# bepu/bepuphysics2

Hardware: NVIDIA H100
Metric: constraint-iterations/sec (solver+integrator) (higher is better)
Workload: dtype f32

## Files before the change

bepuphysics2_b200/csrc/bepu_device_types.h:

```cpp
#pragma once
#include <cuda_runtime.h>
#include <stdint.h>

namespace bepucuda {

constexpr uint32_t kRefIndexMask = 0x0FFFFFFFu;
constexpr uint32_t kRefBundleIntegratesBit = 1u << 28;
constexpr uint32_t kRefIntegrateBit = 1u << 29;
constexpr uint32_t kRefKinematicBit = 1u << 30;
constexpr int32_t kRefEmpty = -1;

struct BodyBuffers {
    float4* pose;
    float4* velocity;
    float4* inertia_local;
    float4* inertia_world;
    const uint8_t* constrained;
    int32_t count;
};

struct DeviceTypeBatch {
    int32_t type_id;
    int32_t bundle_count;
    int32_t device_batch;
    int32_t pad;
    int32_t* refs;
    float* prestep;
    float* impulses;
};

struct FrameParams {
    float dt;
// ... 64 lines not shown
```

bepuphysics2_b200/csrc/bepu_integration.cuh:

```cuda
#pragma once
#include "bepu_device_math.cuh"

namespace BEPU_NS {

BEPU_DI Q4 integrate_orientation(Q4 start, V3 w, float halfDt) {
    float speed = length(w);
    float halfAngle = speed * halfDt;
    float s = sin_approx(halfAngle);
    float scl = s / speed;
    Q4 q{w.x * scl, w.y * scl, w.z * scl, cos_approx(halfAngle)};
    Q4 end = normalize(concatenate(start, q));
    return speed > 1e-15f ? end : start;
}
BEPU_DI Sym3 rotate_inverse_inertia(Sym3 local, Q4 q) { return rotation_sandwich(matrix_from_quaternion(q), local); }
BEPU_DI void callback_integrate_velocity(Velocity& v, float gx, float gy, float gz, float linearDampingDt, float angularDampingDt) {
    v.lin = (v.lin + V3{gx, gy, gz}) * linearDampingDt;
    v.ang = v.ang * angularDampingDt;
}
BEPU_DI void integrate_velocity_extensions(Velocity& v, bool accelerations, V3 linearAcceleration, V3 angularAcceleration, float dt, bool pointGravity, V3 position,
                                           V3 center, float attractorDt) {
    if (accelerations) {
        v.lin = v.lin + linearAcceleration * dt;
        v.ang = v.ang + angularAcceleration * dt;
    }
    if (pointGravity) {
        const V3 offset = position - center;
        const float distance = length(offset);
        const float inverse = 1.0f / fmaxf(1.0f, distance * distance * distance);
        v.lin = v.lin - (offset * attractorDt) * inverse;
// ... 39 lines not shown
```

bepuphysics2_b200/csrc/bepu_layout_kernels.h:

```cpp
#pragma once
#include "bepu_device_types.h"

namespace bepucuda {

void launch_split_bodies(const void* raw, int body_count, const BodyBuffers& B, cudaStream_t s);
void launch_merge_bodies(void* raw, int body_count, const BodyBuffers& B, cudaStream_t s);
struct TransposeDesc {
    int32_t* src_refs;
    float* src_prestep;
    float* src_impulses;
    const int32_t* map;
    int32_t src_count;
    int32_t bodies, prestep_rows, impulse_rows;
    int32_t src_bundle_base;
    int32_t flags;
    const int32_t* features_old;
    const int32_t* features_new;
};
constexpr int32_t kDescResidentImpulses = 1, kDescRedistribute = 2;
enum { kTransposeRefs = 1, kTransposePrestep = 2, kTransposeImpulses = 4 };
void launch_transpose_in_all(const DeviceTypeBatch* tbs, const TransposeDesc* descs, const WorkItem* work, int work_count, int W, int what, cudaStream_t s);
void launch_transpose_out_all(const DeviceTypeBatch* tbs, const TransposeDesc* descs, const WorkItem* work, int work_count, int W, int what, cudaStream_t s);
void launch_fill_i32(int32_t* p, size_t n, int32_t v, cudaStream_t s);
void launch_redistribute_impulses(const DeviceTypeBatch* tbs, const TransposeDesc* descs, const WorkItem* work, int work_count, cudaStream_t s);
// ... 5 lines not shown
    size_t bytes;
};
void launch_batched_copy(const CopyChunk* chunks, int chunk_count, cudaStream_t s);
void launch_ownership_pass1(const DeviceTypeBatch* tbs, const WorkItem* work, int work_count, const int32_t* bodies_per_type, int sync_batch_count, int body_count,
                            int32_t* first_batch, int32_t* sync_refcount, unsigned long long* sync_mask, int32_t* error_flag, cudaStream_t s);
void launch_ownership_rest(const DeviceTypeBatch* tbs, const WorkItem* work, int work_count, const int32_t* bodies_per_type, int body_count, const int32_t* first_batch,
                           const int32_t* sync_refcount, const unsigned long long* sync_mask, uint8_t* constrained, const int32_t* kinematics, int kinematic_count,
                           int32_t* error_flag, const TransposeDesc* descs, int W, int32_t* source_bundle_flags, cudaStream_t s);
void launch_shard_barrier(const ShardPeers& peers, const FrameParams* fp, uint32_t exchange_index, int32_t* error_flag, cudaStream_t s);

void launch_fill_peer_masks(const int32_t* refs, uint32_t* peer_masks, size_t count, const uint8_t* body_masks, int rank, cudaStream_t s);
void launch_boundary_flags(const WorkRecord* records, int count, const int32_t* bodies_per_type, long long peer_delta, uint8_t* flags, cudaStream_t s);

void launch_pack_ref_rows(const WorkRecord* records, int count, int32_t* rows, cudaStream_t s);

constexpr int kLaunchPdl = 1, kLaunchPrefetchRows = 2, kLaunchIntegratorExtensions = 4, kLaunchContactsOnly = 8, kLaunchPrefetchBodies = 16;
struct ShardLaunch {
    ShardPeers peers;
    long long peer_delta;
    ShardStage stage;
};
struct SolverLaunchers {
    void (*constraint_stage)(int stage, const WorkRecord* records, const int32_t* ref_rows, int work_count, const BodyBuffers& B, const FrameParams* fp, int launch_flags,
                             const ShardLaunch* shard, cudaStream_t s);
    void (*kinematic_stage)(int stage, const int32_t* kinematics, int count, const BodyBuffers& B, const FrameParams* fp, int launch_flags, cudaStream_t s);
    void (*final_pose)(const BodyBuffers& B, const FrameParams* fp, int launch_flags, cudaStream_t s);
};
const SolverLaunchers* get_launchers_bepu_fast();
const SolverLaunchers* get_launchers_bepu_strict();

}
// ... 1 lines not shown
```

bepuphysics2_b200/csrc/bepu_solver_kernels.cu:

```cuda
#include <atomic>
#include "bepu_solver_kernels.cuh"
#include "bepu_layout_kernels.h"

namespace BEPU_NS {

using StageLauncher = void(const WorkRecord* records, const int32_t* ref_rows, int work_count, const BodyBuffers& B, const FrameParams* fp, int launch_flags,
                           const ShardLaunch* shard, cudaStream_t s);
StageLauncher launch_stage_warm_start_first, launch_stage_warm_start, launch_stage_solve;

#ifndef BEPU_DEEP_MINB
#define BEPU_DEEP_MINB 12
#endif
constexpr int kDeepBatchBundles = 2150;
#ifndef BEPU_CONTACT_MINB
#define BEPU_CONTACT_MINB 10
#endif
#ifndef BEPU_CONTACT_SOLVE_MINB
#define BEPU_CONTACT_SOLVE_MINB 12
#endif
template <auto Kernel, class... Args>
static void launch_stage_kernel(int work_count, int launch_flags, cudaStream_t s, Args... args) {
    static std::atomic<bool> carveout_set[64] = {};
    int device = 0;
    cudaGetDevice(&device);
    if (!carveout_set[device & 63]) {
        cudaFuncSetAttribute(Kernel, cudaFuncAttributePreferredSharedMemoryCarveout, cudaSharedmemCarveoutMaxShared);
        carveout_set[device & 63] = true;
    }
    const unsigned blocks = (unsigned)(((size_t)work_count * 32 + kStageBlockThreads - 1) / kStageBlockThreads);
    cudaLaunchConfig_t cfg{};
    cfg.gridDim = dim3(blocks);
    cfg.blockDim = dim3(kStageBlockThreads);
    cfg.stream = s;
    cudaLaunchAttribute attr[1];
    attr[0].id = cudaLaunchAttributeProgrammaticStreamSerialization;
    attr[0].val.programmaticStreamSerializationAllowed = 1;
    cfg.attrs = attr;
    cfg.numAttrs = (launch_flags & bepucuda::kLaunchPdl) ? 1 : 0;
    cudaLaunchKernelEx(&cfg, Kernel, args...);
}
template <int STAGE, int MINB, bool kExt, bool kContacts>
static void launch_stage_instance(const WorkRecord* records, const int32_t* ref_rows, int work_count, const BodyBuffers& B, const FrameParams* fp, int launch_flags, const ShardLaunch* shard,
                                  cudaStream_t s) {
    const int flags = ((launch_flags & bepucuda::kLaunchPrefetchRows) ? kStagePrefetchRows : 0) | ((launch_flags & bepucuda::kLaunchPrefetchBodies) ? kStagePrefetchBodies : 0);
    if (!shard) launch_stage_kernel<constraint_stage_kernel<STAGE, MINB, kExt, kContacts>>(work_count, launch_flags, s, records, ref_rows, work_count, B, fp, flags);
    else if constexpr (STAGE != kStageIncremental && !kContacts)
        launch_stage_kernel<constraint_stage_kernel_sharded<STAGE, MINB, kExt>>(work_count, launch_flags, s, records, ref_rows, work_count, B, fp, flags, shard->peers, shard->peer_delta,
                                                                               shard->stage);
}
template <int STAGE, int MINB, bool kContacts>
static void launch_stage_variant(const WorkRecord* records, const int32_t* ref_rows, int work_count, const BodyBuffers& B, const FrameParams* fp, int launch_flags, const ShardLaunch* shard,
                                 cudaStream_t s) {
    if constexpr (STAGE == kStageWarmStartFirst || STAGE == kStageWarmStart) {
        if (launch_flags & bepucuda::kLaunchIntegratorExtensions) return launch_stage_instance<STAGE, MINB, true, kContacts>(records, ref_rows, work_count, B, fp, launch_flags, shard, s);
    }
    launch_stage_instance<STAGE, MINB, false, kContacts>(records, ref_rows, work_count, B, fp, launch_flags, shard, s);
}
template <int STAGE>
static void launch_stage_t(const WorkRecord* records, const int32_t* ref_rows, int work_count, const BodyBuffers& B, const FrameParams* fp, int launch_flags, const ShardLaunch* shard, cudaStream_t s) {
    if constexpr (STAGE != kStageIncremental) {
        if (work_count >= kDeepBatchBundles) return launch_stage_variant<STAGE, BEPU_DEEP_MINB, false>(records, ref_rows, work_count, B, fp, launch_flags, shard, s);
        if (!shard && (launch_flags & bepucuda::kLaunchContactsOnly))
            return launch_stage_variant<STAGE, STAGE == kStageSolve ? BEPU_CONTACT_SOLVE_MINB : BEPU_CONTACT_MINB, true>(records, ref_rows, work_count, B, fp, launch_flags, shard, s);
// ... 53 lines not shown
```

bepuphysics2_b200/csrc/bepu_solver_kernels.cuh:

```cuda
#pragma once
#include "bepu_contacts.cuh"
#include "bepu_joints_more.cuh"
#include "bepu_integration.cuh"
#include "bepu_device_types.h"

namespace BEPU_NS {

using namespace bepucuda;

struct F8 { float a, b, c, d, e, f, g, h; };
#define BEPU_BODY_LD "ld.global.L1::no_allocate.L2::cache_hint.v4.f32"
#define BEPU_BODY_ST "st.global.L1::no_allocate.L2::cache_hint.v4.f32"
BEPU_DI uint64_t l2_evict_last_policy() {
    uint64_t policy;
    asm("createpolicy.fractional.L2::evict_last.b64 %0, 1.0;" : "=l"(policy));
    return policy;
}
BEPU_DI F8 ld256(const float4* p) {
    F8 r;
    asm volatile(BEPU_BODY_LD " {%0,%1,%2,%3}, [%8], %9;\n\t" BEPU_BODY_LD " {%4,%5,%6,%7}, [%8+16], %9;"
                 : "=f"(r.a), "=f"(r.b), "=f"(r.c), "=f"(r.d), "=f"(r.e), "=f"(r.f), "=f"(r.g), "=f"(r.h)
                 : "l"(p), "l"(l2_evict_last_policy())
                 : "memory");
    return r;
// ... 37 lines not shown
}
BEPU_DI void apply_velocity_extensions(const FrameParams& fp, uint32_t idx, V3 position, float dt, float attractorDt, Velocity& v) {
    const float4* accelerations = reinterpret_cast<const float4*>((unsigned long long)fp.accelerations[0] | ((unsigned long long)fp.accelerations[1] << 32));
    v = integrate_velocity_extensions_at(fp.integrate_extensions, accelerations, idx, v.lin, v.ang, dt, position, V3{fp.attractor_center[0], fp.attractor_center[1], fp.attractor_center[2]},
                                         attractorDt);
}

struct EarlyBodies {
    uint32_t slots;
    Inertia inertia[2];
    V3 pos[2];
    Q4 q[2];
};

template <int STAGE, bool NeedsPose, bool kExt>
BEPU_DI void warm_start_body(uint32_t enc, const BodyBuffers& B, const FrameParams& fp, bool early_slot, const EarlyBodies& early, int s, BodyState& b, Velocity& v) {
    const uint32_t idx = enc & kRefIndexMask;
    if (enc & kRefIntegrateBit) {
        Inertia local;
        if (early_slot) {
            local = early.inertia[s];
            b.pos = early.pos[s];
            b.q = early.q[s];
        } else {
            load_inertia(B.inertia_local, idx, local);
            load_pose(B.pose, idx, b.pos, b.q);
        }
        b.inertia.inv_mass = local.inv_mass;
        if (STAGE == kStageWarmStart) {
            b.pos = b.pos + v.lin * fp.dt;
            Q4 previousOrientation = b.q;
            b.q = integrate_orientation(b.q, v.ang, fp.dt * 0.5f);
            b.inertia.t = rotate_inverse_inertia(local.t, b.q);
            if (fp.angular_mode == 1) integrate_angular_conserve_momentum(previousOrientation, local.t, b.inertia.t, v.ang);
            else if (fp.angular_mode == 2) integrate_angular_gyroscopic(b.q, local.t, v.ang, fp.dt);
            store_pose(B.pose, idx, b.pos, b.q);
        } else {
            b.inertia.t = rotate_inverse_inertia(local.t, b.q);
            if (fp.angular_mode == 1) {
                Q4 previousOrientation = integrate_orientation(b.q, v.ang, fp.dt * -0.5f);
                integrate_angular_conserve_momentum(previousOrientation, local.t, b.inertia.t, v.ang);
            } else if (fp.angular_mode == 2) {
                integrate_angular_gyroscopic(b.q, local.t, v.ang, fp.dt);
            }
        }
        callback_integrate_velocity(v, fp.gravity_dt[0], fp.gravity_dt[1], fp.gravity_dt[2], fp.linear_damping_dt, fp.angular_damping_dt);
        if constexpr (kExt) apply_velocity_extensions(fp, idx, b.pos, fp.dt, fp.attractor_dt, v);
        store_inertia(B.inertia_world, idx, b.inertia);
    } else {
        load_inertia(B.inertia_world, idx, b.inertia);
        if (NeedsPose) load_pose(B.pose, idx, b.pos, b.q);
        if (STAGE == kStageWarmStartFirst && fp.angular_mode != 0 && (enc & kRefBundleIntegratesBit) && !(enc & kRefKinematicBit)) {
            Inertia local;
            load_inertia(B.inertia_local, idx, local);
            V3 pos;
            Q4 q;
            load_pose(B.pose, idx, pos, q);
            if (fp.angular_mode == 1) integrate_angular_conserve_momentum(integrate_orientation(q, v.ang, fp.dt * -0.5f), local.t, b.inertia.t, v.ang);
            else integrate_angular_gyroscopic(q, local.t, v.ang, fp.dt);
        }
    }
}
template <int STAGE, bool NeedsPose, bool kExt>
BEPU_DI void gather_for_warm_start(uint32_t enc, const BodyBuffers& B, const FrameParams& fp, bool early_slot, const EarlyBodies& early, int s, BodyState& b, Velocity& v) {
    load_velocity(B.velocity, enc & kRefIndexMask, v);
    warm_start_body<STAGE, NeedsPose, kExt>(enc, B, fp, early_slot, early, s, b, v);
}

template <class T, class PR, class AR> BEPU_DI void call_warm_start(const BodyState* b, PR p, AR a, Velocity* v) {
    if constexpr (T::kNeedsPose) T::warm_start(b, p, a, v);
    else if constexpr (T::kBodies == 2) T::warm_start(b[0].inertia, b[1].inertia, p, a, v[0], v[1]);
    else T::warm_start(b[0].inertia, p, a, v[0]);
}
template <class T, class PR, class AR> BEPU_DI void call_solve(const BodyState* b, float dt, float inverseDt, PR p, AR a, Velocity* v) {
    if constexpr (T::kNeedsPose) T::solve(b, dt, inverseDt, p, a, v);
    else if constexpr (T::kBodies == 2) T::solve(b[0].inertia, b[1].inertia, dt, inverseDt, p, a, v[0], v[1]);
    else T::solve(b[0].inertia, dt, inverseDt, p, a, v[0]);
}
template <class T> BEPU_DI void call_incremental(float dt, const Velocity* v, float* p) {
    if constexpr (T::kIncremental) {
        if constexpr (T::kBodies == 2) T::incremental_update(dt, v[0], v[1], p);
// ... 4 lines not shown
BEPU_DI uint32_t ldg_nc_u32(const void* p) {
    uint32_t v;
    asm volatile("ld.global.nc.u32 %0, [%1];" : "=r"(v) : "l"(p));
    return v;
}
BEPU_DI void push_record(float4* const* arrays, uint32_t mask, uint32_t idx, float a, float b, float c, float d, float e, float f, float g, float h) {
    while (mask) {
        const int q = __ffs((int)mask) - 1;
        mask &= mask - 1u;
        float4* dst = arrays[q] + 2 * (size_t)idx;
        dst[0] = make_float4(a, b, c, d);
        dst[1] = make_float4(e, f, g, h);
    }
}
template <class T, int STAGE, bool kSharded, bool kExt, class PR, class AR>
BEPU_DI void run_lane(const int32_t* refs, PR p, AR a, float* p_rw, uint32_t enc0, uint32_t enc1, const BodyBuffers& B, const FrameParams& fp, const EarlyBodies& early,
                      const ShardPeers* peers = nullptr, long long peer_delta = 0) {
    constexpr int NB = T::kBodies;
    uint32_t enc[NB];
    enc[0] = enc0;
    if constexpr (NB > 1) enc[1] = enc1;
#pragma unroll
    for (int s = 2; s < NB; ++s) enc[s] = (uint32_t)__ldg(refs + s * kLanes);
    uint32_t push_to[kSharded ? NB : 1];
    if constexpr (kSharded) {
#pragma unroll
        for (int s = 0; s < NB; ++s) push_to[s] = peer_delta != 0 ? ldg_nc_u32(refs + peer_delta + s * kLanes) : 0u;
    }
    if ((int32_t)enc[0] == kRefEmpty) return;
    BodyState b[NB];
    Velocity v[NB];
    if constexpr (STAGE == kStageIncremental) {
// ... 14 lines not shown
            }
        }
        rows_ready(p);
        call_solve<T>(b, fp.dt, fp.inverse_dt, p, a, v);
#pragma unroll
        for (int s = 0; s < NB; ++s)
            if (!(enc[s] & kRefKinematicBit)) {
                store_velocity(B.velocity, enc[s] & kRefIndexMask, v[s]);
                if constexpr (kSharded) {
                    const uint32_t mask = push_to[s];
                    if (mask) push_record(peers->velocity, mask, enc[s] & kRefIndexMask, v[s].lin.x, v[s].lin.y, v[s].lin.z, 0.0f, v[s].ang.x, v[s].ang.y, v[s].ang.z, 0.0f);
                }
            }
    } else {
#pragma unroll
        for (int s = 0; s < NB; ++s) gather_for_warm_start<STAGE, T::kNeedsPose, kExt>(enc[s], B, fp, s < 2 && (early.slots >> s & 1u), early, s & 1, b[s], v[s]);
        rows_ready(p);
        call_warm_start<T>(b, p, a, v);
#pragma unroll
        for (int s = 0; s < NB; ++s)
            if (!(enc[s] & kRefKinematicBit)) {
                const uint32_t idx = enc[s] & kRefIndexMask;
                store_velocity(B.velocity, idx, v[s]);
                if constexpr (kSharded) {
                    const uint32_t mask = push_to[s];
                    if (mask) {
                        push_record(peers->velocity, mask, idx, v[s].lin.x, v[s].lin.y, v[s].lin.z, 0.0f, v[s].ang.x, v[s].ang.y, v[s].ang.z, 0.0f);
                        if (enc[s] & kRefIntegrateBit) {
                            const Inertia& in = b[s].inertia;
                            push_record(peers->inertia_world, mask, idx, in.t.xx, in.t.yx, in.t.yy, in.t.zx, in.t.zy, in.t.zz, in.inv_mass, 0.0f);
                            if (STAGE == kStageWarmStart) push_record(peers->pose, mask, idx, b[s].q.x, b[s].q.y, b[s].q.z, b[s].q.w, b[s].pos.x, b[s].pos.y, b[s].pos.z, 0.0f);
// ... 15 lines not shown
    w.refs = reinterpret_cast<int32_t*>((unsigned long long)(unsigned int)lo.x | ((unsigned long long)(unsigned int)lo.y << 32));
    w.prestep = reinterpret_cast<float*>((unsigned long long)(unsigned int)lo.z | ((unsigned long long)(unsigned int)lo.w << 32));
    w.impulses = reinterpret_cast<float*>((unsigned long long)(unsigned int)hi.x | ((unsigned long long)(unsigned int)hi.y << 32));
    w.type_id = hi.z;
    w.live_lanes = hi.w;
    return w;
}

#define BEPU_CONTACT_TYPES(X)                                                                                                     \
    X(0, ConvexOneBody<1>) X(1, ConvexOneBody<2>) X(2, ConvexOneBody<3>) X(3, ConvexOneBody<4>)                                   \
    X(4, ConvexTwoBody<1>) X(5, ConvexTwoBody<2>) X(6, ConvexTwoBody<3>) X(7, ConvexTwoBody<4>)                                   \
    X(8, NonconvexOneBody<2>) X(9, NonconvexOneBody<3>) X(10, NonconvexOneBody<4>)                                                \
    X(15, NonconvexTwoBody<2>) X(16, NonconvexTwoBody<3>) X(17, NonconvexTwoBody<4>)

template <int STAGE, bool kSharded, bool kExt, bool kContacts, class PR, class AR>
BEPU_DI void run_bundle_rows(const WorkRecord& rec, int lane, PR p, AR a, uint32_t enc0, uint32_t enc1, const BodyBuffers& B, const FrameParams& fp, const EarlyBodies& early,
                             const ShardPeers* peers = nullptr, long long peer_delta = 0) {
    const int32_t* refs = rec.refs + lane;
    float* p_rw = rec.prestep + lane;
#define BEPU_CASE(ID, T) \
    case ID: run_lane<T, STAGE, kSharded, kExt>(refs, p, a, p_rw, enc0, enc1, B, fp, early, peers, peer_delta); break;
    if constexpr (kContacts) {
        switch (rec.type_id) {
            BEPU_CONTACT_TYPES(BEPU_CASE)
            default: break;
        }
    } else {
        switch (rec.type_id) {
            BEPU_CONTACT_TYPES(BEPU_CASE)
            BEPU_JOINT_TYPES(BEPU_CASE)
            BEPU_JOINT_TYPES_MORE(BEPU_CASE)
            default: break;
        }
    }
#undef BEPU_CASE
}
template <int STAGE>
BEPU_DI void run_bundle(const WorkRecord& rec, int lane, uint32_t enc0, uint32_t enc1, const BodyBuffers& B, const FrameParams& fp) {
    run_bundle_rows<STAGE, false, false, false>(rec, lane, GlobalRows{rec.prestep + lane}, GlobalAcc{rec.impulses + lane}, enc0, enc1, B, fp, EarlyBodies{});
}
template <int STAGE> BEPU_DI void run_bundle(const WorkRecord& rec, int lane, const BodyBuffers& B, const FrameParams& fp) {
    const uint32_t enc0 = ldg_nc_u32(rec.refs + lane), enc1 = ldg_nc_u32(rec.refs + kLanes + lane);
    run_bundle<STAGE>(rec, lane, enc0, enc1, B, fp);
}

struct StageRowCounts { uint8_t prestep[64], impulses[64], bodies[64], needs_pose[64]; };
__host__ __device__ constexpr StageRowCounts make_stage_row_counts() {
    StageRowCounts c{};
#define BEPU_ROWS(ID, T) \
    c.prestep[ID] = (uint8_t)T::kPrestepRows; c.impulses[ID] = (uint8_t)T::kImpulseRows; c.bodies[ID] = (uint8_t)T::kBodies; c.needs_pose[ID] = T::kNeedsPose ? 1 : 0;
    BEPU_CONTACT_TYPES(BEPU_ROWS)
    BEPU_JOINT_TYPES(BEPU_ROWS)
    BEPU_JOINT_TYPES_MORE(BEPU_ROWS)
#undef BEPU_ROWS
// ... 14 lines not shown
    uint64_t policy;
    asm volatile("createpolicy.fractional.L2::evict_first.b64 %0, 1.0;" : "=l"(policy));
    return policy;
}
BEPU_DI void bulk_copy_g2s(uint32_t dst, const void* src, uint32_t bytes, uint32_t bar, uint64_t policy) {
    asm volatile("cp.async.bulk.shared::cluster.global.mbarrier::complete_tx::bytes.L2::cache_hint [%0], [%1], %2, [%3], %4;" ::"r"(dst), "l"(src), "r"(bytes), "r"(bar),
                 "l"(policy)
                 : "memory");
}

#ifndef BEPU_STAGE_BLOCK_THREADS
#define BEPU_STAGE_BLOCK_THREADS 64
#endif
constexpr int kStageBlockThreads = BEPU_STAGE_BLOCK_THREADS;

constexpr int kStagePrefetchRows = 1, kStagePrefetchBodies = 2;
template <int STAGE, bool kContacts>
BEPU_DI void load_early_bodies(int type_id, uint32_t enc0, uint32_t enc1, const BodyBuffers& B, EarlyBodies& e) {
    if ((int32_t)enc0 == kRefEmpty) return;
    const int bodies = kStageRowCounts.bodies[type_id];
    const bool pose = !kContacts && kStageRowCounts.needs_pose[type_id];
#pragma unroll
    for (int s = 0; s < 2; ++s) {
        const uint32_t enc = s == 0 ? enc0 : enc1;
        const uint32_t idx = enc & kRefIndexMask;
        if (s >= bodies) break;
        if (STAGE == kStageSolve) {
            load_inertia(B.inertia_world, idx, e.inertia[s]);
            if (pose) load_pose(B.pose, idx, e.pos[s], e.q[s]);
            e.slots |= 1u << s;
        } else if (enc & kRefIntegrateBit) {
// ... 9 lines not shown
}
BEPU_DI void shard_wait(const ShardPeers& peers, int lane, uint32_t solve_index, uint32_t exchange_point, int32_t* error_flag) {
    if (lane < peers.rank_count && lane != peers.rank) {
        const unsigned long long* mine = peers.flags[peers.rank];
        const unsigned long long* targets = mine + kShardTargetSlot + (size_t)lane * kShardMaxExchanges;
        const unsigned long long want = (unsigned long long)solve_index * targets[kShardMaxExchanges - 1] + targets[exchange_point];
        unsigned long long seen;
        unsigned int spins = 0;
        do {
            asm volatile("ld.acquire.sys.global.u64 %0, [%1];" : "=l"(seen) : "l"(mine + kShardCounterSlot + lane) : "memory");
        } while (seen < want && ++spins < 100000000u);
        if (seen < want) atomicExch(error_flag, 5);
    }
    __syncwarp();
}
template <int STAGE, bool kSharded, bool kExt, bool kContacts, bool kEarlyBodies>
BEPU_DI void constraint_stage_body(const WorkRecord* __restrict__ records, const int32_t* __restrict__ ref_rows, int work_count, const BodyBuffers& B, const FrameParams* __restrict__ fpp, int flags, const ShardPeers* peers,
                                   long long peer_delta, const ShardStage* shard = nullptr) {
    constexpr bool kStaged = STAGE != kStageIncremental;
    constexpr int kWarps = kStageBlockThreads / 32;
    __shared__ __align__(128) float slab[kStaged ? kWarps * kStageSlabRows * kLanes : 1];
    __shared__ __align__(8) unsigned long long bars[kWarps];
    const int warp_in_block = threadIdx.x >> 5;
    const int global_warp = (blockIdx.x * kStageBlockThreads + threadIdx.x) >> 5;
    const int lane = threadIdx.x & 31;
    WorkRecord rec{};
    uint32_t enc0 = (uint32_t)kRefEmpty, enc1 = 0;
    const int warp = global_warp;
    const bool active = warp < work_count;
    const uint32_t slab_addr = kStaged ? smem_u32(slab) + warp_in_block * kStageSlabBytes : 0;
    const uint32_t bar = smem_u32(&bars[warp_in_block]);
    const bool early_rows = kStaged && (flags & kStagePrefetchRows);
    uint32_t prestep_bytes = 0, impulse_bytes = 0;
    EarlyBodies early{};
    if (active) {
// ... 2 lines not shown
            prestep_bytes = kStageRowCounts.prestep[rec.type_id] * (kLanes * 4);
            impulse_bytes = kStageRowCounts.impulses[rec.type_id] * (kLanes * 4);
            if (lane == 0) {
                mbar_init(bar, 1);
                if (early_rows) {
                    const uint64_t policy = l2_evict_first_policy();
                    mbar_expect_tx(bar, prestep_bytes + impulse_bytes);
                    bulk_copy_g2s(slab_addr, rec.prestep, prestep_bytes, bar, policy);
                    bulk_copy_g2s(slab_addr + prestep_bytes, rec.impulses, impulse_bytes, bar, policy);
                }
            }
        }
        enc0 = ldg_nc_u32(ref_rows + (size_t)warp * (2 * kLanes) + lane);
        enc1 = ldg_nc_u32(ref_rows + (size_t)warp * (2 * kLanes) + kLanes + lane);
        if constexpr (kStaged && kEarlyBodies) {
            if (flags & kStagePrefetchBodies) load_early_bodies<STAGE, kContacts>(rec.type_id, enc0, enc1, B, early);
        }
    }
    const FrameParams fp = *fpp;
    asm volatile("griddepcontrol.wait;" ::: "memory");
    asm volatile("griddepcontrol.launch_dependents;");
    bool boundary = false;
    if constexpr (kSharded) {
        boundary = active && (rec.live_lanes & kRecordBoundaryBit) != 0;
        if (boundary && shard->exchange_index > 0) shard_wait(*peers, lane, fp.shard_solve_index, shard->exchange_index - 1u, shard->error_flag);
    }
    if (!active) return;
    if constexpr (kStaged) {
        if (!early_rows && lane == 0) {
            const uint64_t policy = l2_evict_first_policy();
            mbar_expect_tx(bar, prestep_bytes + impulse_bytes);
            bulk_copy_g2s(slab_addr, rec.prestep, prestep_bytes, bar, policy);
            bulk_copy_g2s(slab_addr + prestep_bytes, rec.impulses, impulse_bytes, bar, policy);
        }
        __syncwarp();
        run_bundle_rows<STAGE, kSharded, kExt, kContacts>(rec, lane, StagedRows{slab_addr + lane * 4, bar, 0u}, StagedAcc{slab_addr + prestep_bytes + lane * 4, rec.impulses + lane}, enc0,
                                                          enc1, B, fp, early, peers, boundary ? peer_delta : 0);
        if constexpr (kSharded) {
            if (boundary) {
                __syncwarp();
                shard_announce(*peers, lane);
            }
        }
    } else {
        run_bundle<STAGE>(rec, lane, enc0, enc1, B, fp);
    }
}

template <int STAGE, int MINB, bool kExt, bool kContacts>
__global__ void __launch_bounds__(kStageBlockThreads, MINB) constraint_stage_kernel(const WorkRecord* __restrict__ records, const int32_t* __restrict__ ref_rows, int work_count, BodyBuffers B, const FrameParams* __restrict__ fpp, int flags) {
    constraint_stage_body<STAGE, false, kExt, kContacts, MINB == 1 || kContacts>(records, ref_rows, work_count, B, fpp, flags, nullptr, 0);
}
// ... 84 lines not shown
```

bepuphysics2_b200/csrc/bepu_topology.cpp:

```cpp
#include "bepu_topology.h"

#include <algorithm>
#include <cstring>
#include <numeric>

#include "../../include/bepucuda.h"

namespace bepucuda {

static TypeInfo make_contact(int bodies, int prestep, int impulses, int contacts, const char* name) {
    TypeInfo t{};
    t.bodies = bodies; t.prestep_rows = prestep; t.impulse_rows = impulses; t.contacts = contacts; t.name = name;
    const int body_rw = 13 + 6;
    t.solve_bytes = 4 * (prestep + 2 * impulses + bodies + bodies * body_rw);
    t.warm_start_bytes = 4 * (prestep + impulses + bodies + bodies * body_rw);
    t.incremental_bytes = 4 * (prestep + contacts + bodies + 6 * bodies);
    return t;
}
static TypeInfo make_joint(int bodies, int prestep, int impulses, int solve_r, int solve_w, int ws_r, int ws_w, const char* name) {
    TypeInfo t{};
    t.bodies = bodies; t.prestep_rows = prestep; t.impulse_rows = impulses; t.contacts = 0; t.name = name;
    t.solve_bytes = 4 * (prestep + 2 * impulses + bodies + solve_r + solve_w);
    t.warm_start_bytes = 4 * (prestep + impulses + bodies + ws_r + ws_w);
    t.incremental_bytes = 0;
// ... 196 lines not shown
    std::vector<StageOp>& ops = prog.ops;
    auto push = [&](int32_t stage, int32_t begin, int32_t count, int32_t exchange, int32_t flags, int64_t bytes) {
        ops.push_back({stage, begin, count, exchange, 0u, flags, bytes});
    };
    auto work_bytes = [&](int32_t begin, int32_t count, int32_t TypeInfo::*per) {
        int64_t bytes = 0;
        for (int32_t w = begin; w < begin + count; ++w)
            bytes += (int64_t)(get_type_info(plan.tbs[(size_t)plan.work[(size_t)w].type_batch].type_id)->*per) * plan.bundle_live[(size_t)w];
        return bytes;
    };
    std::vector<int64_t> warm_start_bytes, solve_bytes;
    for (const TopologyPlan::Batch& bw : plan.batches) {
        warm_start_bytes.push_back(work_bytes(bw.begin, bw.count, &TypeInfo::warm_start_bytes));
        solve_bytes.push_back(work_bytes(bw.begin, bw.count, &TypeInfo::solve_bytes));
    }
    auto batch_stages = [&](int32_t stage) {
        for (size_t b = 0; b < plan.batches.size(); ++b) {
            const TopologyPlan::Batch& bw = plan.batches[b];
            if (bw.count > 0 || (peer_mode && (int)b < plan.sync_batch_count))
                push(stage, bw.begin, bw.count, peer_mode ? (int32_t)b : kNoExchange, bw.contacts_only ? kLaunchContactsOnly : 0,
                     stage == kStageSolve ? solve_bytes[b] : warm_start_bytes[b]);
        }
    };
    const int64_t incremental_bytes = work_bytes(plan.inc_begin, plan.inc_count, &TypeInfo::incremental_bytes);
    const int64_t kinematic_bytes = (int64_t)kinematic_count * 108;
    const int substeps = (int)iterations.size();
    for (int s = 0; s < substeps; ++s) {
        if (s > 0) {
            if (peer_mode) push(kStageKinematic, 0, 0, kRankBarrier, 0, 0);
            if (plan.inc_count > 0) push(kStageIncremental, plan.inc_begin, plan.inc_count, kNoExchange, 0, incremental_bytes);
            if (kinematic_count > 0) push(kStageKinematic, 0, kinematic_count, kNoExchange, 0, kinematic_bytes);
        } else if (integrate_velocity_for_kinematics && kinematic_count > 0) {
            push(kStageKinematicFirst, 0, kinematic_count, kNoExchange, 0, kinematic_bytes);
        }
        if (peer_mode) push(kStageKinematic, 0, 0, kRankBarrier, 0, 0);
        batch_stages(s == 0 ? kStageWarmStartFirst : kStageWarmStart);
        for (int it = 0; it < iterations[(size_t)s]; ++it) batch_stages(kStageSolve);
    }
    if (peer_mode) push(kStageKinematic, 0, 0, kRankBarrier, 0, 0);
    push(kStageFinalPose, 0, body_count, kNoExchange, 0, (int64_t)body_count * 108);

    const StageOp* previous = nullptr;
    for (StageOp& op : ops) {
        op.exchange_index = prog.exchange_count;
        if (op.exchange != kNoExchange) ++prog.exchange_count;
        if (op.exchange == kRankBarrier) continue;
        if (op.stage <= kStageIncremental) {
            if (op.stage != kStageIncremental && previous && previous->stage != kStageIncremental && !(previous->stage <= kStageSolve && previous->work_begin == op.work_begin))
                op.launch_flags |= kLaunchPrefetchRows;
            if (op.stage <= kStageSolve && previous && !(previous->stage <= kStageWarmStart && previous->work_begin == op.work_begin))
                op.launch_flags |= kLaunchPrefetchBodies;
        }
// ... 47 lines not shown
```

bepuphysics2_b200/csrc/bepucuda_api.cu:

```cuda
#include <algorithm>
#include <cmath>
#include <cstring>
#include <string>
#include <vector>

#include "../../include/bepucuda.h"
#include "bepu_layout_kernels.h"
#include "bepu_coloring.h"
#include "bepu_bounds.h"
#include "bepu_topology.h"

using namespace bepucuda;

namespace bepucuda {

struct DeviceBuffer {
    void* ptr = nullptr;
    size_t capacity = 0;
    cudaError_t reserve(size_t bytes) {
        if (bytes <= capacity) return cudaSuccess;
        if (ptr) cudaFree(ptr);
        ptr = nullptr;
        capacity = 0;
        size_t want = bytes + bytes / 4 + 256;
// ... 218 lines not shown
    const int32_t* ref_rows = ctx->ref_rows.as<int32_t>();
    const FrameParams* fp = ctx->frame_params_dev.as<FrameParams>();
    const int32_t* kin = ctx->kinematics_dev.as<int32_t>();
    ShardLaunch shard{ctx->peers, (long long)(ctx->peer32.as<int32_t>() - ctx->refs32.as<int32_t>()), {0, ctx->error_dev.as<int32_t>()}};
    int64_t n = 0;
    const int extensions = integrator_extensions(ctx) ? kLaunchIntegratorExtensions : 0;
    for (size_t i = 0; i < ctx->program.ops.size(); ++i) {
        const StageOp& op = ctx->program.ops[i];
        const bool barrier = op.exchange == kRankBarrier;
        if (barrier || (op.stage == kStageFinalPose ? ctx->B.count > 0 : op.work_count > 0)) {
            if (profile) cudaEventRecord(profile->events[2 * i], s);
            if (barrier) {
                launch_shard_barrier(ctx->peers, fp, op.exchange_index, ctx->error_dev.as<int32_t>(), s);
            } else if (op.stage <= kStageIncremental) {
                shard.stage.exchange_index = op.exchange_index;
                const int flags = (profile ? op.launch_flags & kLaunchContactsOnly : kLaunchPdl | op.launch_flags) | extensions;
                ctx->launchers->constraint_stage(op.stage, records + op.work_begin, ref_rows + (size_t)op.work_begin * 64, op.work_count, ctx->B, fp, flags,
                                                 op.exchange == kNoExchange ? nullptr : &shard, s);
            } else if (op.stage <= kStageKinematic) {
                ctx->launchers->kinematic_stage(op.stage, kin, op.work_count, ctx->B, fp, extensions, s);
            } else {
                ctx->launchers->final_pose(ctx->B, fp, extensions, s);
            }
            if (profile) {
                cudaEventRecord(profile->events[2 * i + 1], s);
                profile->launched[i] = 1;
            }
            ++n;
        }
    }
    if (launches) *launches = n;
// ... 283 lines not shown
    CK(ctx->raw_bodies.reserve(n * 128));
    CK(ctx->pose.reserve(n * 32));
    CK(ctx->velocity.reserve(n * 32));
    CK(ctx->inertia_local.reserve(n * 32));
    CK(ctx->inertia_world.reserve(n * 32));
    const size_t old_constrained_cap = ctx->constrained.capacity;
    CK(ctx->constrained.reserve(n + 1));
    if (ctx->constrained.capacity != old_constrained_cap) CK(cudaMemsetAsync(ctx->constrained.ptr, 0, ctx->constrained.capacity, ctx->stream));
    ctx->body_count = body_count;
    BodyBuffers B{};
    B.pose = ctx->pose.as<float4>();
    B.velocity = ctx->velocity.as<float4>();
    B.inertia_local = ctx->inertia_local.as<float4>();
    B.inertia_world = ctx->inertia_world.as<float4>();
    B.constrained = ctx->constrained.as<uint8_t>();
    B.count = body_count;
    if (B.pose != ctx->B.pose || B.velocity != ctx->B.velocity || B.inertia_local != ctx->B.inertia_local || B.inertia_world != ctx->B.inertia_world ||
        B.constrained != ctx->B.constrained || B.count != ctx->B.count)
        invalidate_graph(ctx);
    ctx->B = B;
    if (body_count > 0) {
        CK(cudaMemcpyAsync(ctx->raw_bodies.ptr, body_dynamics, n * 128, cudaMemcpyHostToDevice, ctx->stream));
        ctx->h2d_accum += (int64_t)n * 128;
        launch_split_bodies(ctx->raw_bodies.ptr, body_count, ctx->B, ctx->stream);
        CK(cudaGetLastError());
    }
    return BEPUCUDA_OK;
}

int32_t bepucuda_begin_constraints(bepucuda_ctx* ctx, int32_t source_bundle_width, int32_t batch_count) {
    if (!ctx || source_bundle_width < 1 || source_bundle_width > 64 || batch_count < 0) return fail(ctx, BEPUCUDA_ERR_INVALID_ARGUMENT, "begin_constraints: bad arguments");
    CK(cudaSetDevice(ctx->device));
    CK(cudaStreamSynchronize(ctx->stream));
// ... 96 lines not shown
    if (!tbs.empty()) CK(cudaMemcpyAsync(ctx->tb_table.ptr, tbs.data(), tbs.size() * sizeof(DeviceTypeBatch), cudaMemcpyHostToDevice, ctx->stream));
    if (!ctx->tdescs.empty()) CK(cudaMemcpyAsync(ctx->tdesc_table.ptr, ctx->tdescs.data(), ctx->tdescs.size() * sizeof(TransposeDesc), cudaMemcpyHostToDevice, ctx->stream));
    if (!topo.work.empty()) CK(cudaMemcpyAsync(ctx->work_table.ptr, topo.work.data(), topo.work.size() * sizeof(WorkItem), cudaMemcpyHostToDevice, ctx->stream));
    if (!ctx->records.empty()) CK(cudaMemcpyAsync(ctx->record_table.ptr, ctx->records.data(), ctx->records.size() * sizeof(WorkRecord), cudaMemcpyHostToDevice, ctx->stream));
    if (!topo.maps.empty()) CK(cudaMemcpyAsync(ctx->map_table.ptr, topo.maps.data(), topo.maps.size() * 4, cudaMemcpyHostToDevice, ctx->stream));
    CK(cudaMemcpyAsync(ctx->bodies_per_type.ptr, bodies_per_type, sizeof(bodies_per_type), cudaMemcpyHostToDevice, ctx->stream));
    if (!ctx->kinematics.empty()) CK(cudaMemcpyAsync(ctx->kinematics_dev.ptr, ctx->kinematics.data(), ctx->kinematics.size() * 4, cudaMemcpyHostToDevice, ctx->stream));

    { int rc = flush_chunks(ctx, ctx->pending_h2d); if (rc != BEPUCUDA_OK) return rc; }
    launch_transpose_in_all(ctx->tb_table.as<DeviceTypeBatch>(), ctx->tdesc_table.as<TransposeDesc>(), ctx->work_table.as<WorkItem>(), topo.all_work_count, W,
                            kTransposeRefs | kTransposePrestep | kTransposeImpulses, ctx->stream);
    const size_t nb = (size_t)std::max(ctx->body_count, 1);
    CK(ctx->first_batch.reserve(nb * 4));
    CK(ctx->sync_refcount.reserve(nb * 4));
    CK(ctx->sync_mask.reserve(nb * 8));
    launch_fill_i32(ctx->first_batch.as<int32_t>(), nb, 0x7fffffff, ctx->stream);
    CK(cudaMemsetAsync(ctx->sync_refcount.ptr, 0, nb * 4, ctx->stream));
    CK(cudaMemsetAsync(ctx->sync_mask.ptr, 0, nb * 8, ctx->stream));
    CK(cudaMemsetAsync(ctx->constrained.ptr, 0, nb, ctx->stream));
    CK(cudaMemsetAsync(ctx->error_dev.ptr, 0, 32, ctx->stream));
    CK(ctx->source_bundle_flags.reserve((size_t)std::max(topo.source_bundles, 1) * 16));
    CK(cudaMemsetAsync(ctx->source_bundle_flags.ptr, 0, (size_t)std::max(topo.source_bundles, 1) * 16, ctx->stream));
    launch_ownership_pass1(ctx->tb_table.as<DeviceTypeBatch>(), ctx->work_table.as<WorkItem>(), topo.all_work_count, ctx->bodies_per_type.as<int32_t>(), topo.sync_batch_count,
                           ctx->body_count, ctx->first_batch.as<int32_t>(), ctx->sync_refcount.as<int32_t>(), (unsigned long long*)ctx->sync_mask.ptr, ctx->error_dev.as<int32_t>(),
                           ctx->stream);
    if (ctx->peer_mode && nb > 0) {
        if ((int)ctx->global_first_batch.size() != ctx->body_count) return fail(ctx, BEPUCUDA_ERR_BAD_STATE, "end_constraints: bepucuda_shard_set_global was not called for this body count");
        CK(cudaMemcpyAsync(ctx->first_batch.ptr, ctx->global_first_batch.data(), (size_t)ctx->body_count * 4, cudaMemcpyHostToDevice, ctx->stream));
    }
    launch_ownership_rest(ctx->tb_table.as<DeviceTypeBatch>(), ctx->work_table.as<WorkItem>(), topo.all_work_count, ctx->bodies_per_type.as<int32_t>(), ctx->body_count,
// ... 526 lines not shown
```

Measured before the change: 2.188 billion.

## Integrate body poses inside incremental stage instead of during warm start

Adds extra blocks to the incremental-contact stage kernel. For every constrained body, these blocks integrate pose and world inertia when angular mode is zero, before the next warm start runs. The warm-start stage then loads the precomputed world inertia and pose instead of doing the orientation integration and inertia rotation serially inside constraint gathering. It can also prefetch early bodies in solve mode. The aim is to take per-body integration off the warm-start critical path and hide it beside the incremental work. The cost is extra blocks and memory traffic, plus correctness depending on first_batch ownership and on the ordering of velocity reads.

```diff
diff --git a/bepuphysics2_b200/csrc/bepu_device_types.h b/bepuphysics2_b200/csrc/bepu_device_types.h
--- a/bepuphysics2_b200/csrc/bepu_device_types.h
+++ b/bepuphysics2_b200/csrc/bepu_device_types.h
@@ -16,6 +16,7 @@
     float4* inertia_local;
     float4* inertia_world;
     const uint8_t* constrained;
+    const int32_t* first_batch;
     int32_t count;
 };
 
diff --git a/bepuphysics2_b200/csrc/bepu_integration.cuh b/bepuphysics2_b200/csrc/bepu_integration.cuh
--- a/bepuphysics2_b200/csrc/bepu_integration.cuh
+++ b/bepuphysics2_b200/csrc/bepu_integration.cuh
@@ -13,6 +13,11 @@
     return speed > 1e-15f ? end : start;
 }
 BEPU_DI Sym3 rotate_inverse_inertia(Sym3 local, Q4 q) { return rotation_sandwich(matrix_from_quaternion(q), local); }
+BEPU_DI void integrate_pose_and_inertia(V3 lin, V3 ang, float dt, Sym3 local, V3& pos, Q4& q, Sym3& world) {
+    pos = pos + lin * dt;
+    q = integrate_orientation(q, ang, dt * 0.5f);
+    world = rotate_inverse_inertia(local, q);
+}
 BEPU_DI void callback_integrate_velocity(Velocity& v, float gx, float gy, float gz, float linearDampingDt, float angularDampingDt) {
     v.lin = (v.lin + V3{gx, gy, gz}) * linearDampingDt;
     v.ang = v.ang * angularDampingDt;
diff --git a/bepuphysics2_b200/csrc/bepu_layout_kernels.h b/bepuphysics2_b200/csrc/bepu_layout_kernels.h
--- a/bepuphysics2_b200/csrc/bepu_layout_kernels.h
+++ b/bepuphysics2_b200/csrc/bepu_layout_kernels.h
@@ -43,7 +43,7 @@
 
 void launch_pack_ref_rows(const WorkRecord* records, int count, int32_t* rows, cudaStream_t s);
 
-constexpr int kLaunchPdl = 1, kLaunchPrefetchRows = 2, kLaunchIntegratorExtensions = 4, kLaunchContactsOnly = 8, kLaunchPrefetchBodies = 16;
+constexpr int kLaunchPdl = 1, kLaunchPrefetchRows = 2, kLaunchIntegratorExtensions = 4, kLaunchContactsOnly = 8, kLaunchPrefetchBodies = 16, kLaunchBodiesIntegrated = 32;
 struct ShardLaunch {
     ShardPeers peers;
     long long peer_delta;
diff --git a/bepuphysics2_b200/csrc/bepu_solver_kernels.cu b/bepuphysics2_b200/csrc/bepu_solver_kernels.cu
--- a/bepuphysics2_b200/csrc/bepu_solver_kernels.cu
+++ b/bepuphysics2_b200/csrc/bepu_solver_kernels.cu
@@ -19,7 +19,7 @@
 #define BEPU_CONTACT_SOLVE_MINB 12
 #endif
 template <auto Kernel, class... Args>
-static void launch_stage_kernel(int work_count, int launch_flags, cudaStream_t s, Args... args) {
+static void launch_stage_kernel(int work_count, unsigned extra_blocks, int launch_flags, cudaStream_t s, Args... args) {
     static std::atomic<bool> carveout_set[64] = {};
     int device = 0;
     cudaGetDevice(&device);
@@ -27,7 +27,7 @@
         cudaFuncSetAttribute(Kernel, cudaFuncAttributePreferredSharedMemoryCarveout, cudaSharedmemCarveoutMaxShared);
         carveout_set[device & 63] = true;
     }
-    const unsigned blocks = (unsigned)(((size_t)work_count * 32 + kStageBlockThreads - 1) / kStageBlockThreads);
+    const unsigned blocks = (unsigned)(((size_t)work_count * 32 + kStageBlockThreads - 1) / kStageBlockThreads) + extra_blocks;
     cudaLaunchConfig_t cfg{};
     cfg.gridDim = dim3(blocks);
     cfg.blockDim = dim3(kStageBlockThreads);
@@ -42,11 +42,14 @@
 template <int STAGE, int MINB, bool kExt, bool kContacts>
 static void launch_stage_instance(const WorkRecord* records, const int32_t* ref_rows, int work_count, const BodyBuffers& B, const FrameParams* fp, int launch_flags, const ShardLaunch* shard,
                                   cudaStream_t s) {
-    const int flags = ((launch_flags & bepucuda::kLaunchPrefetchRows) ? kStagePrefetchRows : 0) | ((launch_flags & bepucuda::kLaunchPrefetchBodies) ? kStagePrefetchBodies : 0);
-    if (!shard) launch_stage_kernel<constraint_stage_kernel<STAGE, MINB, kExt, kContacts>>(work_count, launch_flags, s, records, ref_rows, work_count, B, fp, flags);
+    const bool bodies_integrated = (launch_flags & bepucuda::kLaunchBodiesIntegrated) != 0;
+    const int flags = ((launch_flags & bepucuda::kLaunchPrefetchRows) ? kStagePrefetchRows : 0) | ((launch_flags & bepucuda::kLaunchPrefetchBodies) ? kStagePrefetchBodies : 0) |
+                      (bodies_integrated ? kStageBodiesIntegrated : 0);
+    const unsigned body_blocks = STAGE == kStageIncremental && bodies_integrated ? (unsigned)((B.count + kStageBlockThreads - 1) / kStageBlockThreads) : 0u;
+    if (!shard) launch_stage_kernel<constraint_stage_kernel<STAGE, MINB, kExt, kContacts>>(work_count, body_blocks, launch_flags, s, records, ref_rows, work_count, B, fp, flags);
     else if constexpr (STAGE != kStageIncremental && !kContacts)
-        launch_stage_kernel<constraint_stage_kernel_sharded<STAGE, MINB, kExt>>(work_count, launch_flags, s, records, ref_rows, work_count, B, fp, flags, shard->peers, shard->peer_delta,
-                                                                               shard->stage);
+        launch_stage_kernel<constraint_stage_kernel_sharded<STAGE, MINB, kExt>>(work_count, 0u, launch_flags, s, records, ref_rows, work_count, B, fp, flags, shard->peers,
+                                                                               shard->peer_delta, shard->stage);
 }
 template <int STAGE, int MINB, bool kContacts>
 static void launch_stage_variant(const WorkRecord* records, const int32_t* ref_rows, int work_count, const BodyBuffers& B, const FrameParams* fp, int launch_flags, const ShardLaunch* shard,
diff --git a/bepuphysics2_b200/csrc/bepu_solver_kernels.cuh b/bepuphysics2_b200/csrc/bepu_solver_kernels.cuh
--- a/bepuphysics2_b200/csrc/bepu_solver_kernels.cuh
+++ b/bepuphysics2_b200/csrc/bepu_solver_kernels.cuh
@@ -75,41 +75,47 @@
 };
 
 template <int STAGE, bool NeedsPose, bool kExt>
-BEPU_DI void warm_start_body(uint32_t enc, const BodyBuffers& B, const FrameParams& fp, bool early_slot, const EarlyBodies& early, int s, BodyState& b, Velocity& v) {
+BEPU_DI void warm_start_body(uint32_t enc, const BodyBuffers& B, const FrameParams& fp, bool integrated, bool early_slot, const EarlyBodies& early, int s, BodyState& b,
+                             Velocity& v) {
     const uint32_t idx = enc & kRefIndexMask;
     if (enc & kRefIntegrateBit) {
-        Inertia local;
-        if (early_slot) {
-            local = early.inertia[s];
-            b.pos = early.pos[s];
-            b.q = early.q[s];
+        if (STAGE == kStageWarmStart && !kExt && integrated) {
+            if (early_slot) b.inertia = early.inertia[s];
+            else load_inertia(B.inertia_world, idx, b.inertia);
+            if (NeedsPose) load_pose(B.pose, idx, b.pos, b.q);
         } else {
-            load_inertia(B.inertia_local, idx, local);
-            load_pose(B.pose, idx, b.pos, b.q);
-        }
-        b.inertia.inv_mass = local.inv_mass;
-        if (STAGE == kStageWarmStart) {
-            b.pos = b.pos + v.lin * fp.dt;
-            Q4 previousOrientation = b.q;
-            b.q = integrate_orientation(b.q, v.ang, fp.dt * 0.5f);
-            b.inertia.t = rotate_inverse_inertia(local.t, b.q);
-            if (fp.angular_mode == 1) integrate_angular_conserve_momentum(previousOrientation, local.t, b.inertia.t, v.ang);
-            else if (fp.angular_mode == 2) integrate_angular_gyroscopic(b.q, local.t, v.ang, fp.dt);
-            store_pose(B.pose, idx, b.pos, b.q);
-        } else {
-            b.inertia.t = rotate_inverse_inertia(local.t, b.q);
-            if (fp.angular_mode == 1) {
-                Q4 previousOrientation = integrate_orientation(b.q, v.ang, fp.dt * -0.5f);
-                integrate_angular_conserve_momentum(previousOrientation, local.t, b.inertia.t, v.ang);
-            } else if (fp.angular_mode == 2) {
-                integrate_angular_gyroscopic(b.q, local.t, v.ang, fp.dt);
-            }
+            Inertia local;
+            if (early_slot) {
+                local = early.inertia[s];
+                b.pos = early.pos[s];
+                b.q = early.q[s];
+            } else {
+                load_inertia(B.inertia_local, idx, local);
+                load_pose(B.pose, idx, b.pos, b.q);
+            }
+            b.inertia.inv_mass = local.inv_mass;
+            if (STAGE == kStageWarmStart) {
+                Q4 previousOrientation = b.q;
+                integrate_pose_and_inertia(v.lin, v.ang, fp.dt, local.t, b.pos, b.q, b.inertia.t);
+                if (fp.angular_mode == 1) integrate_angular_conserve_momentum(previousOrientation, local.t, b.inertia.t, v.ang);
+                else if (fp.angular_mode == 2) integrate_angular_gyroscopic(b.q, local.t, v.ang, fp.dt);
+                store_pose(B.pose, idx, b.pos, b.q);
+            } else {
+                b.inertia.t = rotate_inverse_inertia(local.t, b.q);
+                if (fp.angular_mode == 1) {
+                    Q4 previousOrientation = integrate_orientation(b.q, v.ang, fp.dt * -0.5f);
+                    integrate_angular_conserve_momentum(previousOrientation, local.t, b.inertia.t, v.ang);
+                } else if (fp.angular_mode == 2) {
+                    integrate_angular_gyroscopic(b.q, local.t, v.ang, fp.dt);
+                }
+            }
+            store_inertia(B.inertia_world, idx, b.inertia);
         }
         callback_integrate_velocity(v, fp.gravity_dt[0], fp.gravity_dt[1], fp.gravity_dt[2], fp.linear_damping_dt, fp.angular_damping_dt);
         if constexpr (kExt) apply_velocity_extensions(fp, idx, b.pos, fp.dt, fp.attractor_dt, v);
-        store_inertia(B.inertia_world, idx, b.inertia);
     } else {
-        load_inertia(B.inertia_world, idx, b.inertia);
+        if (STAGE == kStageWarmStart && !kExt && early_slot) b.inertia = early.inertia[s];
+        else load_inertia(B.inertia_world, idx, b.inertia);
         if (NeedsPose) load_pose(B.pose, idx, b.pos, b.q);
         if (STAGE == kStageWarmStartFirst && fp.angular_mode != 0 && (enc & kRefBundleIntegratesBit) && !(enc & kRefKinematicBit)) {
             Inertia local;
@@ -123,9 +129,10 @@
     }
 }
 template <int STAGE, bool NeedsPose, bool kExt>
-BEPU_DI void gather_for_warm_start(uint32_t enc, const BodyBuffers& B, const FrameParams& fp, bool early_slot, const EarlyBodies& early, int s, BodyState& b, Velocity& v) {
+BEPU_DI void gather_for_warm_start(uint32_t enc, const BodyBuffers& B, const FrameParams& fp, bool integrated, bool early_slot, const EarlyBodies& early, int s, BodyState& b,
+                                   Velocity& v) {
     load_velocity(B.velocity, enc & kRefIndexMask, v);
-    warm_start_body<STAGE, NeedsPose, kExt>(enc, B, fp, early_slot, early, s, b, v);
+    warm_start_body<STAGE, NeedsPose, kExt>(enc, B, fp, integrated, early_slot, early, s, b, v);
 }
 
 template <class T, class PR, class AR> BEPU_DI void call_warm_start(const BodyState* b, PR p, AR a, Velocity* v) {
@@ -160,8 +167,8 @@
     }
 }
 template <class T, int STAGE, bool kSharded, bool kExt, class PR, class AR>
-BEPU_DI void run_lane(const int32_t* refs, PR p, AR a, float* p_rw, uint32_t enc0, uint32_t enc1, const BodyBuffers& B, const FrameParams& fp, const EarlyBodies& early,
-                      const ShardPeers* peers = nullptr, long long peer_delta = 0) {
+BEPU_DI void run_lane(const int32_t* refs, PR p, AR a, float* p_rw, uint32_t enc0, uint32_t enc1, const BodyBuffers& B, const FrameParams& fp, bool integrated,
+                      const EarlyBodies& early, const ShardPeers* peers = nullptr, long long peer_delta = 0) {
     constexpr int NB = T::kBodies;
     uint32_t enc[NB];
     enc[0] = enc0;
@@ -206,7 +213,7 @@
             }
     } else {
 #pragma unroll
-        for (int s = 0; s < NB; ++s) gather_for_warm_start<STAGE, T::kNeedsPose, kExt>(enc[s], B, fp, s < 2 && (early.slots >> s & 1u), early, s & 1, b[s], v[s]);
+        for (int s = 0; s < NB; ++s) gather_for_warm_start<STAGE, T::kNeedsPose, kExt>(enc[s], B, fp, integrated, s < 2 && (early.slots >> s & 1u), early, s & 1, b[s], v[s]);
         rows_ready(p);
         call_warm_start<T>(b, p, a, v);
 #pragma unroll
@@ -252,12 +259,12 @@
     X(15, NonconvexTwoBody<2>) X(16, NonconvexTwoBody<3>) X(17, NonconvexTwoBody<4>)
 
 template <int STAGE, bool kSharded, bool kExt, bool kContacts, class PR, class AR>
-BEPU_DI void run_bundle_rows(const WorkRecord& rec, int lane, PR p, AR a, uint32_t enc0, uint32_t enc1, const BodyBuffers& B, const FrameParams& fp, const EarlyBodies& early,
-                             const ShardPeers* peers = nullptr, long long peer_delta = 0) {
+BEPU_DI void run_bundle_rows(const WorkRecord& rec, int lane, PR p, AR a, uint32_t enc0, uint32_t enc1, const BodyBuffers& B, const FrameParams& fp, bool integrated,
+                             const EarlyBodies& early, const ShardPeers* peers = nullptr, long long peer_delta = 0) {
     const int32_t* refs = rec.refs + lane;
     float* p_rw = rec.prestep + lane;
 #define BEPU_CASE(ID, T) \
-    case ID: run_lane<T, STAGE, kSharded, kExt>(refs, p, a, p_rw, enc0, enc1, B, fp, early, peers, peer_delta); break;
+    case ID: run_lane<T, STAGE, kSharded, kExt>(refs, p, a, p_rw, enc0, enc1, B, fp, integrated, early, peers, peer_delta); break;
     if constexpr (kContacts) {
         switch (rec.type_id) {
             BEPU_CONTACT_TYPES(BEPU_CASE)
@@ -275,7 +282,7 @@
 }
 template <int STAGE>
 BEPU_DI void run_bundle(const WorkRecord& rec, int lane, uint32_t enc0, uint32_t enc1, const BodyBuffers& B, const FrameParams& fp) {
-    run_bundle_rows<STAGE, false, false, false>(rec, lane, GlobalRows{rec.prestep + lane}, GlobalAcc{rec.impulses + lane}, enc0, enc1, B, fp, EarlyBodies{});
+    run_bundle_rows<STAGE, false, false, false>(rec, lane, GlobalRows{rec.prestep + lane}, GlobalAcc{rec.impulses + lane}, enc0, enc1, B, fp, false, EarlyBodies{});
 }
 template <int STAGE> BEPU_DI void run_bundle(const WorkRecord& rec, int lane, const BodyBuffers& B, const FrameParams& fp) {
     const uint32_t enc0 = ldg_nc_u32(rec.refs + lane), enc1 = ldg_nc_u32(rec.refs + kLanes + lane);
@@ -320,7 +327,7 @@
 #endif
 constexpr int kStageBlockThreads = BEPU_STAGE_BLOCK_THREADS;
 
-constexpr int kStagePrefetchRows = 1, kStagePrefetchBodies = 2;
+constexpr int kStagePrefetchRows = 1, kStagePrefetchBodies = 2, kStageBodiesIntegrated = 4;
 template <int STAGE, bool kContacts>
 BEPU_DI void load_early_bodies(int type_id, uint32_t enc0, uint32_t enc1, const BodyBuffers& B, EarlyBodies& e) {
     if ((int32_t)enc0 == kRefEmpty) return;
@@ -360,11 +367,36 @@
     }
     __syncwarp();
 }
+BEPU_DI void integrate_body_pose(int i, const BodyBuffers& B, const FrameParams* __restrict__ fpp) {
+    const FrameParams fp = *fpp;
+    const bool owned = i < B.count && fp.angular_mode == 0 && (int32_t)ldg_nc_u32(B.first_batch + i) != 0x7fffffff;
+    Inertia local;
+    V3 pos;
+    Q4 q;
+    if (owned) {
+        load_inertia(B.inertia_local, (uint32_t)i, local);
+        load_pose(B.pose, (uint32_t)i, pos, q);
+    }
+    asm volatile("griddepcontrol.wait;" ::: "memory");
+    asm volatile("griddepcontrol.launch_dependents;");
+    if (!owned) return;
+    Velocity v;
+    load_velocity(B.velocity, (uint32_t)i, v);
+    Inertia world;
+    world.inv_mass = local.inv_mass;
+    integrate_pose_and_inertia(v.lin, v.ang, fp.dt, local.t, pos, q, world.t);
+    store_pose(B.pose, (uint32_t)i, pos, q);
+    store_inertia(B.inertia_world, (uint32_t)i, world);
+}
 template <int STAGE, bool kSharded, bool kExt, bool kContacts, bool kEarlyBodies>
 BEPU_DI void constraint_stage_body(const WorkRecord* __restrict__ records, const int32_t* __restrict__ ref_rows, int work_count, const BodyBuffers& B, const FrameParams* __restrict__ fpp, int flags, const ShardPeers* peers,
                                    long long peer_delta, const ShardStage* shard = nullptr) {
     constexpr bool kStaged = STAGE != kStageIncremental;
     constexpr int kWarps = kStageBlockThreads / 32;
+    if constexpr (STAGE == kStageIncremental) {
+        const int bundle_blocks = (work_count + kWarps - 1) / kWarps;
+        if ((int)blockIdx.x >= bundle_blocks) return integrate_body_pose(((int)blockIdx.x - bundle_blocks) * kStageBlockThreads + (int)threadIdx.x, B, fpp);
+    }
     __shared__ __align__(128) float slab[kStaged ? kWarps * kStageSlabRows * kLanes : 1];
     __shared__ __align__(8) unsigned long long bars[kWarps];
     const int warp_in_block = threadIdx.x >> 5;
@@ -397,12 +429,17 @@
         enc0 = ldg_nc_u32(ref_rows + (size_t)warp * (2 * kLanes) + lane);
         enc1 = ldg_nc_u32(ref_rows + (size_t)warp * (2 * kLanes) + kLanes + lane);
         if constexpr (kStaged && kEarlyBodies) {
-            if (flags & kStagePrefetchBodies) load_early_bodies<STAGE, kContacts>(rec.type_id, enc0, enc1, B, early);
+            if (flags & kStagePrefetchBodies) {
+                if (!(flags & kStageBodiesIntegrated)) load_early_bodies<STAGE, kContacts>(rec.type_id, enc0, enc1, B, early);
+                else if (STAGE == kStageWarmStart && kContacts && !kExt && (flags & kStagePrefetchRows) && fpp->angular_mode == 0)
+                    load_early_bodies<kStageSolve, kContacts>(rec.type_id, enc0, enc1, B, early);
+            }
         }
     }
     const FrameParams fp = *fpp;
     asm volatile("griddepcontrol.wait;" ::: "memory");
     asm volatile("griddepcontrol.launch_dependents;");
+    const bool integrated = STAGE == kStageWarmStart && !kExt && (flags & kStageBodiesIntegrated) && fp.angular_mode == 0;
     bool boundary = false;
     if constexpr (kSharded) {
         boundary = active && (rec.live_lanes & kRecordBoundaryBit) != 0;
@@ -418,7 +455,7 @@
         }
         __syncwarp();
         run_bundle_rows<STAGE, kSharded, kExt, kContacts>(rec, lane, StagedRows{slab_addr + lane * 4, bar, 0u}, StagedAcc{slab_addr + prestep_bytes + lane * 4, rec.impulses + lane}, enc0,
-                                                          enc1, B, fp, early, peers, boundary ? peer_delta : 0);
+                                                          enc1, B, fp, integrated, early, peers, boundary ? peer_delta : 0);
         if constexpr (kSharded) {
             if (boundary) {
                 __syncwarp();
diff --git a/bepuphysics2_b200/csrc/bepu_topology.cpp b/bepuphysics2_b200/csrc/bepu_topology.cpp
--- a/bepuphysics2_b200/csrc/bepu_topology.cpp
+++ b/bepuphysics2_b200/csrc/bepu_topology.cpp
@@ -234,28 +234,30 @@
         warm_start_bytes.push_back(work_bytes(bw.begin, bw.count, &TypeInfo::warm_start_bytes));
         solve_bytes.push_back(work_bytes(bw.begin, bw.count, &TypeInfo::solve_bytes));
     }
-    auto batch_stages = [&](int32_t stage) {
+    auto batch_stages = [&](int32_t stage, int32_t flags) {
         for (size_t b = 0; b < plan.batches.size(); ++b) {
             const TopologyPlan::Batch& bw = plan.batches[b];
             if (bw.count > 0 || (peer_mode && (int)b < plan.sync_batch_count))
-                push(stage, bw.begin, bw.count, peer_mode ? (int32_t)b : kNoExchange, bw.contacts_only ? kLaunchContactsOnly : 0,
+                push(stage, bw.begin, bw.count, peer_mode ? (int32_t)b : kNoExchange, flags | (bw.contacts_only ? kLaunchContactsOnly : 0),
                      stage == kStageSolve ? solve_bytes[b] : warm_start_bytes[b]);
         }
     };
+    const int32_t bodies_integrated = plan.inc_count > 0 && !peer_mode ? kLaunchBodiesIntegrated : 0;
     const int64_t incremental_bytes = work_bytes(plan.inc_begin, plan.inc_count, &TypeInfo::incremental_bytes);
     const int64_t kinematic_bytes = (int64_t)kinematic_count * 108;
     const int substeps = (int)iterations.size();
     for (int s = 0; s < substeps; ++s) {
         if (s > 0) {
             if (peer_mode) push(kStageKinematic, 0, 0, kRankBarrier, 0, 0);
-            if (plan.inc_count > 0) push(kStageIncremental, plan.inc_begin, plan.inc_count, kNoExchange, 0, incremental_bytes);
+            if (plan.inc_count > 0) push(kStageIncremental, plan.inc_begin, plan.inc_count, kNoExchange, bodies_integrated, incremental_bytes);
             if (kinematic_count > 0) push(kStageKinematic, 0, kinematic_count, kNoExchange, 0, kinematic_bytes);
         } else if (integrate_velocity_for_kinematics && kinematic_count > 0) {
             push(kStageKinematicFirst, 0, kinematic_count, kNoExchange, 0, kinematic_bytes);
         }
         if (peer_mode) push(kStageKinematic, 0, 0, kRankBarrier, 0, 0);
-        batch_stages(s == 0 ? kStageWarmStartFirst : kStageWarmStart);
-        for (int it = 0; it < iterations[(size_t)s]; ++it) batch_stages(kStageSolve);
+        if (s == 0) batch_stages(kStageWarmStartFirst, 0);
+        else batch_stages(kStageWarmStart, bodies_integrated);
+        for (int it = 0; it < iterations[(size_t)s]; ++it) batch_stages(kStageSolve, 0);
     }
     if (peer_mode) push(kStageKinematic, 0, 0, kRankBarrier, 0, 0);
     push(kStageFinalPose, 0, body_count, kNoExchange, 0, (int64_t)body_count * 108);
diff --git a/bepuphysics2_b200/csrc/bepucuda_api.cu b/bepuphysics2_b200/csrc/bepucuda_api.cu
--- a/bepuphysics2_b200/csrc/bepucuda_api.cu
+++ b/bepuphysics2_b200/csrc/bepucuda_api.cu
@@ -256,7 +256,8 @@
                 launch_shard_barrier(ctx->peers, fp, op.exchange_index, ctx->error_dev.as<int32_t>(), s);
             } else if (op.stage <= kStageIncremental) {
                 shard.stage.exchange_index = op.exchange_index;
-                const int flags = (profile ? op.launch_flags & kLaunchContactsOnly : kLaunchPdl | op.launch_flags) | extensions;
+                const int op_flags = extensions ? op.launch_flags & ~kLaunchBodiesIntegrated : op.launch_flags;
+                const int flags = (profile ? op_flags & (kLaunchContactsOnly | kLaunchBodiesIntegrated) : kLaunchPdl | op_flags) | extensions;
                 ctx->launchers->constraint_stage(op.stage, records + op.work_begin, ref_rows + (size_t)op.work_begin * 64, op.work_count, ctx->B, fp, flags,
                                                  op.exchange == kNoExchange ? nullptr : &shard, s);
             } else if (op.stage <= kStageKinematic) {
@@ -570,9 +571,10 @@
     B.inertia_local = ctx->inertia_local.as<float4>();
     B.inertia_world = ctx->inertia_world.as<float4>();
     B.constrained = ctx->constrained.as<uint8_t>();
+    B.first_batch = ctx->first_batch.as<int32_t>();
     B.count = body_count;
     if (B.pose != ctx->B.pose || B.velocity != ctx->B.velocity || B.inertia_local != ctx->B.inertia_local || B.inertia_world != ctx->B.inertia_world ||
-        B.constrained != ctx->B.constrained || B.count != ctx->B.count)
+        B.constrained != ctx->B.constrained || B.first_batch != ctx->B.first_batch || B.count != ctx->B.count)
         invalidate_graph(ctx);
     ctx->B = B;
     if (body_count > 0) {
@@ -699,6 +701,7 @@
     CK(ctx->first_batch.reserve(nb * 4));
     CK(ctx->sync_refcount.reserve(nb * 4));
     CK(ctx->sync_mask.reserve(nb * 8));
+    ctx->B.first_batch = ctx->first_batch.as<int32_t>();
     launch_fill_i32(ctx->first_batch.as<int32_t>(), nb, 0x7fffffff, ctx->stream);
     CK(cudaMemsetAsync(ctx->sync_refcount.ptr, 0, nb * 4, ctx->stream));
     CK(cudaMemsetAsync(ctx->sync_mask.ptr, 0, nb * 8, ctx->stream));
```

Result: faster. 2.319 billion, median of 6 (+6.0%).
